# hellojialee/OffsetGuided

Measured on AMD Instinct MI355X. Metric: images/sec end-to-end (backbone+decode) @640x640 bs8; decoder-only ms/img, higher is better.
Workload: dtype f16

## Files before the change

### offsetguided_amd/csrc/conv3x3.hip

```cpp
#include <stdio.h>
#include <stdlib.h>

#include <type_traits>

#include "lp_dtype.h"
#include "og_common.h"

namespace {

typedef lp8 bf16x8;
typedef float f32x4 __attribute__((ext_vector_type(4)));
typedef unsigned short u16x4 __attribute__((ext_vector_type(4)));
typedef unsigned short u16x8 __attribute__((ext_vector_type(8)));

constexpr int kZeroPageBytes = 256;

struct ConvArgs {
    const unsigned short *x;
    const unsigned short *w;
    const float *bias;
    const unsigned short *skip;
    unsigned short *out;
    unsigned short *up;
    float *partial;
    int *counters;
    const unsigned short *zero;
    int N, H, W, Cin, Cout, M;
    int Hin, Win, stride, taps;
    int n_tiles, steps_per_split, ksplit, relu;
    const unsigned short *x2;
    int Cin2, H2, W2, stride2, steps_main, steps_total, w_row;
    uint32_t magic_w, magic_h, magic_chunks;
    int x_bytes, w_bytes;
    unsigned long long *stamps;
    OgWarm warm;
};

#if defined(OG_TILED_STAMPS) || defined(OG_PW_STAMPS)
#ifndef OG_DEBUG_STAMPS
#define OG_DEBUG_STAMPS 1
#endif
#endif
#ifdef OG_DEBUG_STAMPS
#define CONV_STAMP(i)                                                                                         \
    do {                                                                                                      \
        if (a.stamps && tid == 0)                                                                             \
            a.stamps[((size_t)blockIdx.y * gridDim.x + blockIdx.x) * 8 + (i)] = __builtin_amdgcn_s_memrealtime(); \
    } while (0)
#else
#define CONV_STAMP(i) do { } while (0)
#endif

__device__ __forceinline__ unsigned short f2bf(float f) { return f2lp(f); }
__device__ __forceinline__ float bf2f(unsigned short u) { return lp2f(u); }

__device__ __forceinline__ void glds16(const void *g, unsigned char *l)
{
    __builtin_amdgcn_global_load_lds((const __attribute__((address_space(1))) void *)g,
                                     (__attribute__((address_space(3))) void *)l, 16, 0, 0);
}

__device__ __forceinline__ void blds16(__amdgpu_buffer_rsrc_t r, uint32_t voff, uint32_t soff, unsigned char *l)
{
    __builtin_amdgcn_raw_ptr_buffer_load_lds(r, (__attribute__((address_space(3))) void *)l, 16, voff, soff, 0, 0);
}
constexpr uint32_t kOobOffset = 0x80000000u;

__device__ __forceinline__ void store_b128_sc1(__amdgpu_buffer_rsrc_t r, uint32_t voff, uint32_t soff, f32x4 v)
{
    asm volatile("buffer_store_dwordx4 %0, %1, %2, %3 offen sc1\n\ts_nop 1" ::"v"(v), "v"(voff), "s"(r), "s"(soff) : "memory");
}

template <int N>
__device__ __forceinline__ void wait_vm_lgkm0()
{
    __builtin_amdgcn_s_waitcnt((N & 15) | (7 << 4) | (0 << 8) | ((N >> 4) << 14));
    asm volatile("" ::: "memory");
}

__device__ __forceinline__ uint32_t div_magic(uint32_t n, uint32_t magic) { return magic ? __umulhi(n, magic) : n; }

template <int BM, int BN>
struct EpiloguePre {
    f32x4 bias[BN / 32];
    u16x4 skip[BM / 32][BN / 32];
};

template <int BM, int BN>
__device__ __forceinline__ void epilogue_load(EpiloguePre<BM, BN> &pre, const ConvArgs &a, int m0, int n0, int wave, int lane)
{
    constexpr int MT = BM / 32, NT = BN / 32;
    const int wm = wave >> 1, wn = wave & 1;
#pragma unroll
    for (int n = 0; n < NT; ++n)
        pre.bias[n] = *reinterpret_cast<const f32x4 *>(a.bias + n0 + wn * (BN / 2) + n * 16 + (lane >> 4) * 4);
#pragma unroll
    for (int m = 0; m < MT; ++m) {
        const int pm = m0 + wm * (BM / 2) + m * 16 + (lane & 15);
#pragma unroll
        for (int n = 0; n < NT; ++n) {
            const int co = n0 + wn * (BN / 2) + n * 16 + (lane >> 4) * 4;
            pre.skip[m][n] = (u16x4){0, 0, 0, 0};
            if (a.skip && pm < a.M) pre.skip[m][n] = *reinterpret_cast<const u16x4 *>(a.skip + (size_t)pm * a.Cout + co);
        }
    }
}

template <int BM, int BN>
__device__ __forceinline__ void epilogue_finish(const f32x4 (&acc)[BN / 32][BM / 32], const EpiloguePre<BM, BN> &pre,
                                                const ConvArgs &a, int m0, int n0, int wave, int lane)
{
    constexpr int MT = BM / 32, NT = BN / 32;
    const int wm = wave >> 1, wn = wave & 1;
#pragma unroll
    for (int m = 0; m < MT; ++m) {
        const int pm = m0 + wm * (BM / 2) + m * 16 + (lane & 15);
        if (pm >= a.M) continue;
#pragma unroll
// ... 446 lines not shown
    OG_REQUIRE(x2, OG_EINVAL, "og_conv2d_proj: null pointer");
    Proj pj;
    pj.x2 = x2; pj.H2 = H2; pj.W2 = W2; pj.Cin2 = Cin2; pj.stride2 = stride2;
    return conv_run(OG_LP_STR("og_conv2d_proj"), x, w_cat, bias, nullptr, out, N, Hin, Win, Cin, Cout, ksize, stride, relu, workspace,
                    workspace_bytes, stream, pj);
}

#ifndef OG_DT_F16
OG_API int og_conv3x3s2_tiled_supported(int N, int H, int W, int Cin, int Cout)
{
    if (N <= 0 || H <= 0 || W <= 0 || Cin <= 0 || Cout <= 0 || (H & 1) || (W & 1)) return 0;
    if ((long)N * H * W * Cin >= (1l << 30) || (long)N * H * W * Cout >= (1l << 32)) return 0;
    if (Cout % 128 || Cin % 64) return 0;
    return ((H / 2) % 8 == 0 && (W / 2) % 16 == 0) ? 1 : ((W / 2) == 40 && (H / 2) % 2 == 0) ? 2 : 0;
}

OG_API int og_conv3x3_tiled_supported(int N, int H, int W, int Cin, int Cout)
{
    if (N <= 0 || H <= 0 || W <= 0 || Cin <= 0 || Cout <= 0) return 0;
    if ((long)N * H * W * Cin >= (1l << 30) || (long)N * H * W * Cout >= (1l << 30)) return 0;
    return tiled_kind(H, W, Cin, Cout);
}

OG_API size_t og_conv3x3_tiled_workspace_bytes(int N, int H, int W, int Cin, int Cout)
{
    const int kind = og_conv3x3_tiled_supported(N, H, W, Cin, Cout);
    if (!kind) return 0;
    const long items = tiled_items(kind, N, H, W, Cout);
    const int ks = tiled_ksplit(kind, items, Cin);
    if (ks <= 1 || items > (long)kMaxTiles) return 0;
    return kZeroPageBytes + kMaxTiles * sizeof(int) + (size_t)items * ks * tiled_slab_bytes(kind);
}

OG_API int og_conv3x3_pack_w16(const void *w, int Cin, int Cout, int order, void *packed, void *stream)
{
    OG_REQUIRE(order >= 0 && order <= 3, OG_EINVAL,
               "og_conv3x3_pack_w16: order is 0 / 1 (3x3, stride 1 / 2) or 2 / 3 (1x1, cout tiles of 128 / 64)");
    OG_REQUIRE(w && packed, OG_EINVAL, "og_conv3x3_pack_w16: null pointer");
    OG_REQUIRE(Cin > 0 && Cout > 0 && Cin % 64 == 0 && Cout % (order == 3 ? 64 : 128) == 0, OG_EUNSUPPORTED,
               "og_conv3x3_pack_w16: Cin must be a multiple of 64 and Cout of %d (got %d -> %d)", order == 3 ? 64 : 128, Cin, Cout);
    const long slots = (long)Cout * (order >= 2 ? 1 : 9) * Cin / 8;
    hipLaunchKernelGGL(conv3x3_pack_kernel, dim3((unsigned)((slots + 255) / 256)), dim3(256), 0, (hipStream_t)stream,
                       (const unsigned short *)w, (unsigned short *)packed, Cin, Cout, order);
    OG_LAUNCH_CHECK("og_conv3x3_pack_w16");
    return OG_OK;
}
#endif

namespace {
int conv3x3_tiled_impl(const char *name, const void *x, const void *w_packed, const float *bias, const void *skip, void *out, void *up,
                       int N, int H, int W, int Cin, int Cout, int relu, void *workspace, size_t workspace_bytes, void *stream)
{
    const OgWarm warm = og_take_warm_hint();
    OG_REQUIRE(x && w_packed && bias && (out || up), OG_EINVAL, "%s: null pointer", name);
    OG_REQUIRE(!up || (uintptr_t)up % 16 == 0, OG_EINVAL, "%s: `up` must be 16-byte aligned", name);
    OG_REQUIRE(N > 0 && H > 0 && W > 0, OG_EINVAL, "%s: bad shape", name);
    const long M = (long)N * H * W;
    OG_REQUIRE(M * (long)Cin < (1l << 30) && M * (long)Cout < (1l << 30), OG_EUNSUPPORTED, "%s: tensor too large (>= 2 GiB)", name);
    const int kind = tiled_kind(H, W, Cin, Cout);
    OG_REQUIRE(kind != 0, OG_EUNSUPPORTED, "%s: needs Cout %% 128 == 0, Cin %% 64 == 0 and H, W multiples of 16 or W == 40 with H %% 4 == 0 "
               "(got %dx%d, %d -> %d)", name, H, W, Cin, Cout);
    ConvArgs h = {};
    h.x = (const unsigned short *)x; h.w = (const unsigned short *)w_packed; h.bias = bias;
    h.skip = (const unsigned short *)skip; h.out = (unsigned short *)out; h.up = (unsigned short *)up;
    h.N = N; h.H = H; h.W = W; h.Cin = Cin; h.Cout = Cout; h.M = (int)M; h.n_tiles = Cout / 128; h.relu = relu;
    h.Hin = H; h.Win = W; h.stride = 1; h.taps = 9;
    h.x_bytes = (int)(M * Cin * 2);
    h.w_bytes = Cout * 9 * Cin * 2;
#ifdef OG_TILED_STAMPS
    h.stamps = g_stamps;
#endif
    hipStream_t st = (hipStream_t)stream;
    h.warm = warm;
    const long items = tiled_items(kind, N, H, W, Cout);
    h.ksplit = (items <= (long)kMaxTiles) ? tiled_ksplit(kind, items, Cin) : 1;
    if (h.ksplit > 1) {
        const size_t need = kZeroPageBytes + kMaxTiles * sizeof(int) + (size_t)items * h.ksplit * tiled_slab_bytes(kind);
        OG_REQUIRE(workspace && workspace_bytes >= need, OG_ENOSPC, "%s: workspace %zu < %zu bytes (og_conv3x3_tiled_workspace_bytes)", name,
                   workspace ? workspace_bytes : (size_t)0, need);
        OG_REQUIRE((uintptr_t)workspace % 256 == 0, OG_EINVAL, "%s: workspace must be 256-byte aligned", name);
        h.counters = (int *)((char *)workspace + kZeroPageBytes);
        h.partial = (float *)((char *)workspace + kZeroPageBytes + kMaxTiles * sizeof(int));
    }
#define TILED_LAUNCH(TW_, TH_, WM_, VAR_)                                                                             \
    do {                                                                                                              \
        constexpr int halo_ = ((TW_ + 2) * (TH_ + 2) * 5 * 16 + 1023) / 1024 * 1024;                                  \
        const int lds_ = 2 * halo_ + (TW_ == 20 ? OG_TILED_RING20 : TW_ == 40 ? OG_TILED_RING40 : 3) * 128 * 64 + 1024; \
        static OgAttrOnce attr_;                                                                                      \
        if (attr_.need())                                                                                             \
            (void)hipFuncSetAttribute((const void *)conv3x3_tiled_kernel<TW_, TH_, WM_, VAR_, 4>,                     \
                                      hipFuncAttributeMaxDynamicSharedMemorySize, 160 * 1024);                        \
        const long blocks_ = (long)N * (H / TH_) * (W / TW_) * h.n_tiles * h.ksplit;                                  \
        hipLaunchKernelGGL((conv3x3_tiled_kernel<TW_, TH_, WM_, VAR_, 4>), dim3((unsigned)blocks_), dim3(256), lds_, st, h); \
    } while (0)
#ifndef OG_TILED_VAR16
#define OG_TILED_VAR16 26
#endif
    if (kind == 1) TILED_LAUNCH(16, 16, 4, OG_TILED_VAR16);
    else if (kind == 3) TILED_LAUNCH(20, 4, 1, 2);
    else TILED_LAUNCH(40, 4, 2, 2);
#undef TILED_LAUNCH
    OG_LAUNCH_CHECK(name);
    return OG_OK;
}
}

OG_API int OG_LP_NAME(og_conv3x3_tiled)(const void *x, const void *w_packed, const float *bias, const void *skip, void *out, int N,
                                        int H, int W, int Cin, int Cout, int relu, void *workspace, size_t workspace_bytes,
                                        void *stream)
{
    return conv3x3_tiled_impl(OG_LP_STR("og_conv3x3_tiled"), x, w_packed, bias, skip, out, nullptr, N, H, W, Cin, Cout, relu, workspace,
                              workspace_bytes, stream);
}

OG_API int OG_LP_NAME(og_conv3x3_tiled_up2)(const void *x, const void *w_packed, const float *bias, const void *skip, void *up, int N,
                                            int H, int W, int Cin, int Cout, int relu, void *workspace, size_t workspace_bytes,
                                            void *stream)
{
    const char *name = OG_LP_STR("og_conv3x3_tiled_up2");
    OG_REQUIRE(up, OG_EINVAL, "%s: null pointer", name);
    OG_REQUIRE((long)N * H * W * 4 * Cout < (1l << 30), OG_EUNSUPPORTED, "%s: tensor too large (>= 2 GiB)", name);
    return conv3x3_tiled_impl(name, x, w_packed, bias, skip, nullptr, up, N, H, W, Cin, Cout, relu, workspace, workspace_bytes, stream);
}

OG_API int OG_LP_NAME(og_conv3x3s2_tiled)(const void *x, const void *w_packed, const float *bias, const void *skip, void *out,
                                          int N, int Hin, int Win, int Cin, int Cout, int relu, void *stream)
{
    const char *name = OG_LP_STR("og_conv3x3s2_tiled");
    OG_REQUIRE(x && w_packed && bias && out, OG_EINVAL, "%s: null pointer", name);
    OG_REQUIRE(N > 0 && Hin > 0 && Win > 0 && !(Hin & 1) && !(Win & 1), OG_EINVAL, "%s: bad shape", name);
    const int H = Hin / 2, W = Win / 2;
    const long M = (long)N * H * W, Min = (long)N * Hin * Win;
    OG_REQUIRE(Min * (long)Cin < (1l << 30) && M * (long)Cout < (1l << 30), OG_EUNSUPPORTED, "%s: tensor too large (>= 2 GiB)", name);
    const int kind = og_conv3x3s2_tiled_supported(N, Hin, Win, Cin, Cout);
    OG_REQUIRE(kind != 0, OG_EUNSUPPORTED,
               "%s: needs Cout %% 128 == 0, Cin %% 64 == 0 and an output of 8k x 16k pixels or 2k x 40 (got %dx%d -> %dx%d, %d -> %d)", name,
               Hin, Win, H, W, Cin, Cout);
    ConvArgs h = {};
    h.warm = og_take_warm_hint();
    h.x = (const unsigned short *)x; h.w = (const unsigned short *)w_packed; h.bias = bias;
    h.skip = (const unsigned short *)skip; h.out = (unsigned short *)out;
    h.N = N; h.H = H; h.W = W; h.Cin = Cin; h.Cout = Cout; h.M = (int)M; h.n_tiles = Cout / 128; h.relu = relu;
    h.Hin = Hin; h.Win = Win; h.stride = 2; h.taps = 9;
    h.x_bytes = (int)(Min * Cin * 2);
    h.w_bytes = Cout * 9 * Cin * 2;
    constexpr int lds_ = 3 * 128 * 64 + 3 * 3 * 4096;
#define S2_LAUNCH(TW_, TH_, WM_, VAR_)                                                                                \
    do {                                                                                                              \
        static OgAttrOnce attr_;                                                                                      \
        if (attr_.need())                                                                                             \
            (void)hipFuncSetAttribute((const void *)conv3x3s2_tiled_kernel<TW_, TH_, WM_, VAR_>,                      \
                                      hipFuncAttributeMaxDynamicSharedMemorySize, lds_);                              \
        const long blocks_ = (long)N * (H / TH_) * (W / TW_) * h.n_tiles;                                             \
        hipLaunchKernelGGL((conv3x3s2_tiled_kernel<TW_, TH_, WM_, VAR_>), dim3((unsigned)blocks_), dim3(256), lds_,   \
                           (hipStream_t)stream, h);                                                                   \
    } while (0)
    if (kind == 2) S2_LAUNCH(40, 2, 1, 2);
    else S2_LAUNCH(16, 8, 2, 2);
#undef S2_LAUNCH
    OG_LAUNCH_CHECK(name);
    return OG_OK;
}

static int pw_fill(const char *name, PwArgs &a, const void *x1, int C1, int H1, int W1, int s1, const void *x2, int C2, int H2, int W2,
                   int s2, const void *w_packed, const float *bias, int N, int H, int W, int Cout, int bn)
{
    OG_REQUIRE(x1 && w_packed, OG_EINVAL, "%s: null pointer", name);
    OG_REQUIRE(N > 0 && H > 0 && W > 0 && (s1 == 1 || s1 == 2) && (!x2 || s2 == 1 || s2 == 2), OG_EINVAL, "%s: bad shape", name);
    OG_REQUIRE(C1 > 0 && C1 % 64 == 0 && (!x2 || (C2 > 0 && C2 % 64 == 0)) && Cout % bn == 0, OG_EUNSUPPORTED,
               "%s: input channels must be multiples of 64 and Cout of %d (got %d + %d -> %d)", name, bn, C1, x2 ? C2 : 0, Cout);
    OG_REQUIRE((H - 1) * s1 < H1 && (W - 1) * s1 < W1, OG_EINVAL, "%s: the strided output reaches outside the input", name);
    OG_REQUIRE(!x2 || (C2 == C1 && H2 == H1 && W2 == W1 && s2 == s1), OG_EUNSUPPORTED,
               "%s: a second input must have the shape and stride of the first", name);
    const long M = (long)N * H * W;
    OG_REQUIRE((long)N * H1 * W1 * C1 < (1l << 30) && (!x2 || (long)N * H2 * W2 * C2 < (1l << 30)) && M * Cout < (1l << 30), OG_EUNSUPPORTED,
// ... 82 lines not shown
```

### offsetguided_amd/csrc/conv3x3_tiled.inc

```

template <int N, int I = 0, class F>
__device__ __forceinline__ void og_static_for(F &&f)
{
    if constexpr (I < N) {
        f(std::integral_constant<int, I>());
        og_static_for<N, I + 1>(f);
    }
}

__host__ __device__ __forceinline__ constexpr int tiled_swz(int row) { return (4 - ((row >> 2) & 3)) & 3; }

__global__ void __launch_bounds__(256)
conv3x3_pack_kernel(const unsigned short *w, unsigned short *packed, int Cin, int Cout, int order)
{
    const long slot = (long)blockIdx.x * 256 + threadIdx.x;
    const int taps = order >= 2 ? 1 : 9, rows = order == 3 ? 64 : 128;
    const long total = (long)Cout * taps * Cin / 8;
    if (slot >= total) return;
    const int chunks = Cin >> 5;
    const int in_stage = (int)(slot % (rows * 4));
    long stage = slot / (rows * 4);
    const int kS2[9] = {0, 2, 6, 8, 3, 5, 1, 7, 4};
    const int tslot = (int)(stage % taps), tap = order == 1 ? kS2[tslot] : tslot;
    stage /= taps;
    const int q = (int)(stage % chunks), nt = (int)(stage / chunks);
    const int r = in_stage >> 2, jp = in_stage & 3, j = jp ^ tiled_swz(r);
    const unsigned short *src = w + ((size_t)(nt * rows + r) * taps + tap) * Cin + q * 32;
    u16x8 v;
#pragma unroll
    for (int e = 0; e < 8; ++e) v[e] = src[order >= 2 ? 8 * j + e : (e < 4 ? 4 * j + e : 16 + 4 * j + (e - 4))];
    *reinterpret_cast<u16x8 *>(packed + slot * 8) = v;
}

template <int TW, int TH, int WM, int VAR, int NW>
__device__ __forceinline__ void conv3x3_tiled_body(const ConvArgs &a, const int bid, const int nblk)
{
    constexpr int BN = 128, WN = NW / WM, kThr = 64 * NW, kPieceB = kThr * 16;
    constexpr int kHaloW = TW + 2, kHaloPx = (TW + 2) * (TH + 2), kPitch = 80;
    constexpr int NPA = (kHaloPx * 5 + kThr - 1) / kThr;
    constexpr int kABytes = (kHaloPx * 5 * 16 + 1023) / 1024 * 1024, kBBytes = BN * 64;
#ifndef OG_TILED_RING20
#define OG_TILED_RING20 6
#endif
#ifndef OG_TILED_RING40
#define OG_TILED_RING40 4
#endif
    constexpr int kRing = TW == 20 ? OG_TILED_RING20 : TW == 40 ? OG_TILED_RING40 : 3;
    constexpr bool kWfRot = TW == 16 && (VAR & 16) != 0;
    constexpr bool kWfAhead = kRing > 3 || kWfRot;
    constexpr int kAhead = kWfAhead ? kRing : kRing - 1;
    constexpr int kWin = kWfAhead ? kAhead - 2 : kAhead - 1;
    static_assert(kRing == 3 || kRing == 4 || kRing == 6 || kRing == 9, "ring sizes the slot arithmetic serves");
    constexpr int kDump = kRing * kBBytes + 2 * kABytes;
    constexpr int PW = kBBytes / kPieceB;
    constexpr int MT = TW * TH / 16 / WM, NT = 8 / WN;
    static_assert(TW * TH % (16 * WM) == 0 && NW % WM == 0 && 8 % WN == 0 && PW >= 1, "unsupported tile");
    static_assert(NPA <= 8 - kWin, "the last halo piece must be older than everything tap 8's wait leaves in flight (the steps 8 - kWin .. 7)");
    static_assert(kDump + 1024 <= 80 * 1024, "two workgroups per CU");
    extern __shared__ __attribute__((aligned(1024))) unsigned char lds[];
    unsigned char *const bufB = lds, *const bufA = lds + kRing * kBBytes;

    const int tid = threadIdx.x, wave = tid >> 6, lane = tid & 63;
    const unsigned warm_v = og_warm_touch(a.warm, (unsigned)bid * kThr + (unsigned)tid);
#ifdef OG_TILED_STAMPS
    {
        unsigned long long rt_entry;
        asm volatile("s_memrealtime %0\n\ts_waitcnt lgkmcnt(0)" : "=s"(rt_entry));
        if (a.stamps) a.stamps[((size_t)blockIdx.x * 4 + wave) * 16 + 7] = rt_entry;
    }
#endif
    const int wid = ((nblk & 7) == 0 && !(VAR & 4)) ? og_xcd_remap(bid, nblk) : bid;
    const int ksplit = a.ksplit, item = wid / ksplit, split = wid - item * ksplit;
    const int tiles_x = a.W / TW, tiles_y = a.H / TH, chunks = a.Cin >> 5;
    const int q0 = split * (chunks / ksplit), q_end = q0 + chunks / ksplit;
    const int nt_i = item % a.n_tiles;
    int t = item / a.n_tiles;
    const int tx = t % tiles_x;
    t /= tiles_x;
    const int ty = t % tiles_y, img = t / tiles_y;
    const int n0 = nt_i * BN;

    const __amdgpu_buffer_rsrc_t xr = __builtin_amdgcn_make_buffer_rsrc(const_cast<unsigned short *>(a.x), 0, a.x_bytes, 0x00020000);
    const __amdgpu_buffer_rsrc_t wr = __builtin_amdgcn_make_buffer_rsrc(const_cast<unsigned short *>(a.w), 0, a.w_bytes, 0x00020000);
    uint32_t a_off[NPA];
#pragma unroll
    for (int i = 0; i < NPA; ++i) {
        const int p = tid + kThr * i, hp = p / 5, c = p - hp * 5;
        const int hy = hp / kHaloW, hx = hp - hy * kHaloW;
        const int gy = ty * TH - 1 + hy, gx = tx * TW - 1 + hx;
        const bool ok = c < 4 && hp < kHaloPx && gy >= 0 && gy < a.H && gx >= 0 && gx < a.W;
        a_off[i] = ok ? (uint32_t)((((img * a.H + gy) * a.W + gx) * a.Cin + c * 8) * 2) : kOobOffset;
    }
    const int piece = wave * 64 * 16;
    const uint32_t w_voff = (uint32_t)tid * 16;
    const uint32_t w_tile = (uint32_t)nt_i * (uint32_t)(chunks * 9 * kBBytes);
    auto issue_a = [&](int i, int q, int buf) {
        const int blk = i * kPieceB + piece;
        blds16(xr, a_off[i], q * 64, blk < kABytes ? bufA + buf * kABytes + blk : lds + kDump);
    };
    int ring_lo = 0, ring_hi = 2 * kBBytes;
    auto ring_off = [&](int slot) { return kRing == 4 ? (slot < 2 ? ring_lo : ring_hi) + (slot & 1) * kBBytes : slot * kBBytes; };
    auto issue_b = [&](int step, int ring_bytes) {
#pragma unroll
        for (int i = 0; i < PW; ++i)
            blds16(wr, w_voff, w_tile + step * kBBytes + i * kPieceB, bufB + ring_bytes + piece + i * kPieceB);
    };

    const int wm = wave / WN, wn = wave % WN;
    const int fcol = lane & 15, fk = lane >> 4;
    const int w_rd = ((wn * NT) * 16 + fcol) * 64 + ((fk ^ tiled_swz(fcol)) << 4);
    int px_off[MT];
#pragma unroll
    for (int m = 0; m < MT; ++m) {
        const int lp = (wm * MT + m) * 16 + fcol;
        px_off[m] = ((lp / TW) * kHaloW + lp % TW) * kPitch + fk * 8;
    }

    typedef unsigned long long u64;
    typedef u64 u64x2 __attribute__((ext_vector_type(2)));
    const uint32_t lds_a = (uint32_t)(uintptr_t)(__attribute__((address_space(3))) unsigned char *)bufA;
    uint32_t px_addr[TW == 16 ? 1 : MT];
#pragma unroll
    for (int m = 0; m < (TW == 16 ? 1 : MT); ++m) px_addr[m] = lds_a + px_off[m];
    auto read_px1 = [&](auto m_tag, auto off_tag, uint32_t buf_off, bf16x8 (&pf)[MT]) {
        constexpr int OFF = decltype(off_tag)::value, m = decltype(m_tag)::value;
        constexpr int imm = OFF + (TW == 16 ? m * kHaloW * kPitch : 0);
        const uint32_t addr = px_addr[TW == 16 ? 0 : m] + buf_off;
        u64 lo, hi;
        asm volatile("ds_read_b64 %0, %1 offset:%2" : "=v"(lo) : "v"(addr), "i"(imm));
        asm volatile("ds_read_b64 %0, %1 offset:%2" : "=v"(hi) : "v"(addr), "i"(imm + 32));
        u64x2 v;
        v[0] = lo;
        v[1] = hi;
        pf[m] = __builtin_bit_cast(bf16x8, v);
    };
    auto read_px = [&](auto off_tag, uint32_t buf_off, bf16x8 (&pf)[MT]) {
        og_static_for<MT>([&](auto m_tag) { read_px1(m_tag, off_tag, buf_off, pf); });
    };

    f32x4 acc[NT][MT];
    if (a.skip && split == 0) {
        static_assert(NT % 2 == 0, "cout blocks in pairs");
        u16x8 sk2[NT / 2][MT];
#pragma unroll
        for (int m = 0; m < MT; ++m) {
            const int lp = (wm * MT + m) * 16 + fcol;
            const size_t opx = (size_t)(img * a.H + ty * TH + lp / TW) * a.W + tx * TW + lp % TW;
#pragma unroll
            for (int np = 0; np < NT / 2; ++np)
                sk2[np][m] = __builtin_nontemporal_load(reinterpret_cast<const u16x8 *>(a.skip + opx * a.Cout + n0 + (wn * NT + 2 * np + (fk & 1)) * 16 + (fk >> 1) * 8));
        }
#pragma unroll
        for (int i = 0; i < NPA; ++i) issue_a(i, q0, 0);
#pragma unroll
        for (int i = 0; i < kAhead; ++i) issue_b(9 * q0 + i, (i % kRing) * kBBytes);
#pragma unroll
        for (int np = 0; np < NT / 2; ++np)
#pragma unroll
            for (int m = 0; m < MT; ++m) {
                typedef uint32_t u32x4s __attribute__((ext_vector_type(4)));
                typedef uint32_t u32x2s __attribute__((ext_vector_type(2)));
                const u32x4s v = __builtin_bit_cast(u32x4s, sk2[np][m]);
                const auto r0 = __builtin_amdgcn_permlane16_swap(v[0], v[2], false, false);
                const auto r1 = __builtin_amdgcn_permlane16_swap(v[1], v[3], false, false);
                const u16x4 lo = __builtin_bit_cast(u16x4, (u32x2s){r0[0], r1[0]}), hi = __builtin_bit_cast(u16x4, (u32x2s){r0[1], r1[1]});
                acc[2 * np][m] = (f32x4){bf2f(lo[0]), bf2f(lo[1]), bf2f(lo[2]), bf2f(lo[3])};
                acc[2 * np + 1][m] = (f32x4){bf2f(hi[0]), bf2f(hi[1]), bf2f(hi[2]), bf2f(hi[3])};
            }
    } else {
#pragma unroll
        for (int i = 0; i < NPA; ++i) issue_a(i, q0, 0);
#pragma unroll
        for (int i = 0; i < kAhead; ++i) issue_b(9 * q0 + i, (i % kRing) * kBBytes);
#pragma unroll
        for (int n = 0; n < NT; ++n)
#pragma unroll
            for (int m = 0; m < MT; ++m) acc[n][m] = (f32x4){0.f, 0.f, 0.f, 0.f};
    }

    constexpr int kSets = NT == 8 ? 9 : NT == 4 ? 6 : 3, kFree = kSets - NT;
    static_assert(!kWfRot || ((18 * NT) % kSets == 0 && kFree >= 1 && NT * (MT - 1) >= kFree + 1 + MT), "rotating fragment sets");
    bf16x8 pf[2][MT], wf[kWfAhead && !kWfRot ? 2 : 1][kWfRot ? kSets : NT];
#ifdef OG_TILED_STAMPS
    unsigned long long st_end, st_w, st_b, st_prev;
    uint32_t sum_wait = 0, sum_bar = 0, sum_body = 0, n_st = 0;
    {
        unsigned long long mt0, rt0;
        asm volatile("s_memtime %0\n\ts_memrealtime %1\n\ts_waitcnt lgkmcnt(0)" : "=s"(mt0), "=s"(rt0));
        st_end = st_w = st_b = st_prev = mt0;
        if (a.stamps) {
            a.stamps[((size_t)blockIdx.x * 4 + wave) * 16 + 4] = mt0;
            a.stamps[((size_t)blockIdx.x * 4 + wave) * 16 + 5] = rt0;
        }
    }
#endif
    wait_vm_lgkm0<(kAhead - 1) * PW>();
    __builtin_amdgcn_s_barrier();
    asm volatile("" ::: "memory");
#ifdef OG_TILED_STAMPS
    {
        unsigned long long rt_first;
        asm volatile("s_memrealtime %0\n\ts_waitcnt lgkmcnt(0)" : "=s"(rt_first));
        if (a.stamps) a.stamps[((size_t)blockIdx.x * 4 + wave) * 16 + 9] = rt_first;
    }
#endif
    read_px(std::integral_constant<int, 0>(), 0u, pf[0]);
    if constexpr (kWfAhead) {
#pragma unroll
        for (int n = 0; n < NT; ++n) wf[0][n] = *reinterpret_cast<const bf16x8 *>(bufB + w_rd + n * 1024);
    }

    auto chunk_body = [&](auto more_tag, auto par_tag, int q) {
        constexpr bool MORE = decltype(more_tag)::value;
        constexpr int PAR = decltype(par_tag)::value;
        const uint32_t cur_off = (uint32_t)((q & 1) * kABytes), nxt_off = (uint32_t)(((q + 1) & 1) * kABytes);
        og_static_for<9>([&](auto tap_tag) {
            constexpr int tap = decltype(tap_tag)::value;
            constexpr int kSlot0 = kRing == 6 ? 3 * PAR : kRing == 4 ? PAR : 0;
            const int s = q * 9 + tap;
            {
                constexpr int kYounger = [] {
                    int n = 0;
                    for (int j = 1; j <= kWin; ++j) {
                        const int t = tap - j;
                        if (t < 0) n += PW;
                        else n += ((MORE && t < NPA) ? 1 : 0) + ((MORE || t + kAhead < 9) ? PW : 0);
                    }
                    return n;
                }();
                wait_vm_lgkm0<kYounger>();
            }
#ifdef OG_TILED_STAMPS
            asm volatile("" : "+s"(st_end), "+s"(st_w), "+s"(st_b));
            sum_wait += (uint32_t)st_w - (uint32_t)st_prev;
            sum_bar += (uint32_t)st_b - (uint32_t)st_w;
            sum_body += (uint32_t)st_end - (uint32_t)st_b;
            st_prev = st_end;
            ++n_st;
            asm volatile("s_memtime %0" : "=s"(st_w));
#endif
            __builtin_amdgcn_s_barrier();
#ifdef OG_TILED_STAMPS
            asm volatile("s_memtime %0" : "=s"(st_b));
#endif
            __builtin_amdgcn_sched_barrier(0);
            auto issue_dma = [&]() {
                if (MORE && tap < NPA) issue_a(tap, q + 1, (q + 1) & 1);
                if (MORE || tap + kAhead < 9) issue_b(s + kAhead, ring_off((kSlot0 + tap + kAhead) % kRing));
            };
            const unsigned char *wB = bufB + ring_off((kSlot0 + tap + (kWfAhead ? 1 : 0)) % kRing);
            constexpr int wcur = kWfAhead ? (PAR + tap) & 1 : 0, wnxt = kWfAhead ? (PAR + tap + 1) & 1 : 0;
            if constexpr (kWfRot) {
                constexpr bool kNext = MORE || tap < 8;
                constexpr int t18 = PAR * 9 + tap, cur = (PAR + tap) & 1, nxt = cur ^ 1;
                if (!(VAR & 1)) __builtin_amdgcn_s_setprio(1);
                og_static_for<NT * MT>([&](auto i_tag) {
                    constexpr int i = decltype(i_tag)::value, n = i / MT, m = i % MT;
                    acc[n][m] = OG_LP_MFMA(wf[0][(t18 * NT + n) % kSets], pf[cur][m], acc[n][m]);
                    if constexpr (m == MT - 1) {
                        constexpr int j = n + kFree;
                        if constexpr (j < NT && kNext)
                            wf[0][((t18 + 1) * NT + j) % kSets] = *reinterpret_cast<const bf16x8 *>(wB + w_rd + j * 1024);
                    } else {
                        constexpr int k = n * (MT - 1) + m;
                        if constexpr (k < kFree) {
                            if constexpr (kNext) wf[0][((t18 + 1) * NT + k) % kSets] = *reinterpret_cast<const bf16x8 *>(wB + w_rd + k * 1024);
                        } else if constexpr (k == kFree) {
                            issue_dma();
                        } else if constexpr (k - kFree - 1 < MT) {
                            constexpr int pm = k - kFree - 1;
                            if constexpr (tap < 8)
                                read_px1(std::integral_constant<int, pm>(), std::integral_constant<int, (((tap + 1) / 3) * kHaloW + (tap + 1) % 3) * kPitch>(),
                                         cur_off, pf[nxt]);
                            else if constexpr (MORE)
                                read_px1(std::integral_constant<int, pm>(), std::integral_constant<int, 0>(), nxt_off, pf[nxt]);
                        }
                    }
                    __builtin_amdgcn_sched_barrier(0);
                });
                if (!(VAR & 1)) __builtin_amdgcn_s_setprio(0);
            } else if constexpr (kWfAhead) {
                static_assert(NT * MT >= 1 + MT + NT, "an MFMA gap per issue item");
                constexpr bool kNext = MORE || tap < 8;
                constexpr int cur = (PAR + tap) & 1, nxt = cur ^ 1;
                if (!(VAR & 1)) __builtin_amdgcn_s_setprio(1);
                og_static_for<NT * MT>([&](auto i_tag) {
                    constexpr int i = decltype(i_tag)::value, n = i / MT, m = i % MT;
                    acc[n][m] = OG_LP_MFMA(wf[wcur][n], pf[cur][m], acc[n][m]);
                    if constexpr (i == 0) {
                        issue_dma();
                    } else if constexpr (i - 1 < MT) {
                        if constexpr (tap < 8)
                            read_px1(std::integral_constant<int, i - 1>(), std::integral_constant<int, (((tap + 1) / 3) * kHaloW + (tap + 1) % 3) * kPitch>(),
                                     cur_off, pf[nxt]);
                        else if constexpr (MORE)
                            read_px1(std::integral_constant<int, i - 1>(), std::integral_constant<int, 0>(), nxt_off, pf[nxt]);
                    } else if constexpr (i - 1 - MT < NT) {
                        if constexpr (kNext) wf[wnxt][i - 1 - MT] = *reinterpret_cast<const bf16x8 *>(wB + w_rd + (i - 1 - MT) * 1024);
                    }
                    __builtin_amdgcn_sched_barrier(0);
                });
                if (!(VAR & 1)) __builtin_amdgcn_s_setprio(0);
            } else {
            if (!(VAR & 2)) issue_dma();
            if constexpr (tap < 8)
                read_px(std::integral_constant<int, (((tap + 1) / 3) * kHaloW + (tap + 1) % 3) * kPitch>(), cur_off, pf[(PAR + tap + 1) & 1]);
            else if constexpr (MORE)
                read_px(std::integral_constant<int, 0>(), nxt_off, pf[(PAR + tap + 1) & 1]);
#pragma unroll
            for (int n = 0; n < NT; ++n) wf[0][n] = *reinterpret_cast<const bf16x8 *>(wB + w_rd + n * 1024);
            if (VAR & 2) issue_dma();
            if (!(VAR & 1)) __builtin_amdgcn_s_setprio(1);
#pragma unroll
            for (int n = 0; n < NT; ++n)
#pragma unroll
                for (int m = 0; m < MT; ++m) acc[n][m] = OG_LP_MFMA(wf[wcur][n], pf[(PAR + tap) & 1][m], acc[n][m]);
            if (!(VAR & 1)) __builtin_amdgcn_s_setprio(0);
            }
#ifdef OG_TILED_STAMPS
            asm volatile("s_memtime %0" : "=s"(st_end));
#endif
        });
    };
    const std::true_type yes;
    const std::false_type no;
    const std::integral_constant<int, 0> even;
    const std::integral_constant<int, 1> odd;
    int q = q0;
#pragma unroll 1
    for (; q + 2 < q_end; q += 2) {
        chunk_body(yes, even, q);
        chunk_body(yes, odd, q + 1);
        if constexpr (kRing == 4) {
            const int t = ring_lo;
            ring_lo = ring_hi;
            ring_hi = t;
        }
    }
    chunk_body(yes, even, q);
    chunk_body(no, odd, q + 1);

#ifdef OG_TILED_STAMPS
    {
        unsigned long long mt1, rt1;
        asm volatile("s_waitcnt lgkmcnt(0)\n\ts_memtime %0\n\ts_memrealtime %1\n\ts_waitcnt lgkmcnt(0)" : "=s"(mt1), "=s"(rt1));
        asm volatile("" : "+s"(st_end), "+s"(st_w), "+s"(st_b));
        sum_wait += (uint32_t)st_w - (uint32_t)st_prev;
        sum_bar += (uint32_t)st_b - (uint32_t)st_w;
        sum_body += (uint32_t)st_end - (uint32_t)st_b;
        if (a.stamps && lane == 0) {
            unsigned long long *o = a.stamps + ((size_t)blockIdx.x * 4 + wave) * 16;
            o[0] = sum_wait; o[1] = sum_bar; o[2] = sum_body; o[3] = n_st; o[12] = mt1; o[6] = rt1;
            o[10] = __builtin_amdgcn_s_getreg((4) | (0 << 6) | (31 << 11));
            o[11] = __builtin_amdgcn_s_getreg((20) | (0 << 6) | (31 << 11));
        }
    }
#endif
    if (ksplit > 1) {
        typedef uint32_t u32x4 __attribute__((ext_vector_type(4)));
        constexpr int F = NT * MT;
        constexpr uint32_t kSlabBytes = F * kThr * 16;
        uint64_t slab_base = reinterpret_cast<uint64_t>(a.partial) + (uint64_t)item * ksplit * kSlabBytes;
        slab_base = ((uint64_t)(uint32_t)__builtin_amdgcn_readfirstlane((int)(slab_base >> 32)) << 32) |
                    (uint64_t)(uint32_t)__builtin_amdgcn_readfirstlane((int)(uint32_t)slab_base);
        const __amdgpu_buffer_rsrc_t slabs = __builtin_amdgcn_make_buffer_rsrc(
            reinterpret_cast<char *>(slab_base), 0, __builtin_amdgcn_readfirstlane((int)(ksplit * kSlabBytes)), 0x00020000);
        const uint32_t own_off = __builtin_amdgcn_readfirstlane(split * kSlabBytes);
#pragma unroll
        for (int n = 0; n < NT; ++n)
#pragma unroll
            for (int m = 0; m < MT; ++m)
                store_b128_sc1(slabs, (n * MT + m) * kThr * 16 + tid * 16, own_off, acc[n][m]);
        asm volatile("s_waitcnt vmcnt(0)" ::: "memory");
        __syncthreads();
        int *flag = reinterpret_cast<int *>(lds);
        if (tid == 0) {
            const int old = __hip_atomic_fetch_add(a.counters + item, 1, __ATOMIC_RELAXED, __HIP_MEMORY_SCOPE_AGENT);
            const int last = old == ksplit - 1;
            if (last) __hip_atomic_store(a.counters + item, 0, __ATOMIC_RELAXED, __HIP_MEMORY_SCOPE_AGENT);
            *flag = last;
        }
        __syncthreads();
        if (!*flag) return;
#pragma unroll
        for (int n = 0; n < NT; ++n)
#pragma unroll
            for (int m = 0; m < MT; ++m) acc[n][m] = (f32x4){0.f, 0.f, 0.f, 0.f};
        for (int sp = 0; sp < ksplit; ++sp) {
            const uint32_t soff = __builtin_amdgcn_readfirstlane(sp * kSlabBytes);
            f32x4 part[F];
#pragma unroll
            for (int i = 0; i < F; ++i)
                part[i] = __builtin_bit_cast(f32x4, __builtin_amdgcn_raw_buffer_load_b128(slabs, i * kThr * 16 + tid * 16, soff, 16));
#pragma unroll
            for (int n = 0; n < NT; ++n)
#pragma unroll
                for (int m = 0; m < MT; ++m) acc[n][m] += part[n * MT + m];
        }
    }

    constexpr int kOPitch = BN * 2 + 16, kTilePx = TW * TH, kPerPx = BN / 8;
    static_assert(kTilePx * kOPitch <= kDump + 1024, "output staging must fit the LDS of the main loop");
    f32x4 bias_r[NT];
#pragma unroll
    for (int n = 0; n < NT; ++n) bias_r[n] = *reinterpret_cast<const f32x4 *>(a.bias + n0 + (wn * NT + n) * 16 + fk * 4);
    __syncthreads();
#pragma unroll
    for (int m = 0; m < MT; ++m) {
        const int px = (wm * MT + m) * 16 + fcol;
#pragma unroll
        for (int n = 0; n < NT; ++n) {
            const int cl = (wn * NT + n) * 16 + fk * 4;
            const f32x4 v = acc[n][m] + bias_r[n];
            u16x4 o;
#pragma unroll
            for (int jj = 0; jj < 4; ++jj) o[jj] = f2bf(a.relu ? fmaxf(v[jj], 0.f) : v[jj]);
            *reinterpret_cast<u16x4 *>(lds + px * kOPitch + cl * 2) = o;
        }
    }
    __syncthreads();
    if (a.up) {
        const int W2 = 2 * a.W;
        const size_t up_tile = ((size_t)img * 2 * a.H + 2 * ty * TH) * W2 + 2 * tx * TW;
        constexpr int kPieces = kTilePx * kPerPx;
        static_assert(kPieces % kThr == 0, "whole rounds");
        for (int g0 = tid; g0 < kPieces; g0 += 2 * kThr) {
            u16x8 lo[2], hi[2][4];
            size_t off[2];
#pragma unroll
            for (int u = 0; u < 2; ++u) {
                const int g = min(g0 + u * kThr, kPieces - kThr + tid), px = g / kPerPx, cg = g % kPerPx;
                off[u] = (up_tile + (size_t)(2 * (px / TW)) * W2 + 2 * (px % TW)) * a.Cout + n0 + cg * 8;
#pragma unroll
                for (int q = 0; q < 4; ++q)
                    hi[u][q] = *reinterpret_cast<const u16x8 *>(a.up + off[u] + ((size_t)(q >> 1) * W2 + (q & 1)) * a.Cout);
                lo[u] = *reinterpret_cast<const u16x8 *>(lds + px * kOPitch + cg * 16);
            }
#pragma unroll
            for (int u = 0; u < 2; ++u)
#pragma unroll
                for (int q = 0; q < 4; ++q) {
                    if (u == 1 && g0 + kThr >= kPieces) continue;
                    u16x8 o;
#pragma unroll
                    for (int j = 0; j < 8; ++j) o[j] = f2bf(bf2f(hi[u][q][j]) + bf2f(lo[u][j]));
                    *reinterpret_cast<u16x8 *>(a.up + off[u] + ((size_t)(q >> 1) * W2 + (q & 1)) * a.Cout) = o;
                }
        }
    } else {
        const size_t tile_px = (size_t)(img * a.H + ty * TH) * a.W + tx * TW;
        for (int g = tid; g < kTilePx * kPerPx; g += kThr) {
            const int px = g / kPerPx, cg = g % kPerPx;
            const size_t off = (tile_px + (size_t)(px / TW) * a.W + (px % TW)) * a.Cout + n0 + cg * 8;
            *reinterpret_cast<u16x8 *>(a.out + off) = *reinterpret_cast<const u16x8 *>(lds + px * kOPitch + cg * 16);
        }
    }
#ifdef OG_TILED_STAMPS
    if (a.stamps && lane == 0) {
        unsigned long long rt_end;
        asm volatile("s_memrealtime %0\n\ts_waitcnt lgkmcnt(0)" : "=s"(rt_end));
        a.stamps[((size_t)blockIdx.x * 4 + wave) * 16 + 8] = rt_end;
    }
#endif
    og_warm_sink(warm_v);
}

template <int TW, int TH, int WM, int VAR = 0, int NW = 4>
__global__ void __launch_bounds__(64 * NW, NW / 2)
conv3x3_tiled_kernel(ConvArgs a)
{
    conv3x3_tiled_body<TW, TH, WM, VAR, NW>(a, blockIdx.x, gridDim.x);
}

template <int TW, int TH, int WM, int VAR = 0>
__global__ void __launch_bounds__(256, 2)
conv3x3s2_tiled_kernel(ConvArgs a)
{
    constexpr int BN = 128, WN = 4 / WM;
    constexpr bool kRowFrag = TW == 16;
    constexpr int kPitch = 80, kImgPx = (TW + 1) * (TH + 1);
    constexpr int NPA = (kImgPx * 5 + 255) / 256;
    constexpr int kABytes = NPA * 256 * 16, kBBytes = BN * 64, kRing = 3;
    constexpr int PW = kBBytes / (256 * 16);
    constexpr int MT = TW * TH / 16 / WM, NT = 8 / WN;
    static_assert(TW * TH % (16 * WM) == 0 && 4 % WM == 0, "unsupported tile");
    static_assert(NPA == 3, "the static halo schedule below issues three pieces per phase image");
    static_assert(kRing * kBBytes + 3 * kABytes <= 80 * 1024, "two workgroups per CU");
    extern __shared__ __attribute__((aligned(1024))) unsigned char lds[];
    unsigned char *const bufB = lds, *const bufA = lds + kRing * kBBytes;

    const int tid = threadIdx.x, wave = tid >> 6, lane = tid & 63;
    const unsigned warm_v = og_warm_touch(a.warm, blockIdx.x * 256u + (unsigned)tid);
    const int nblk = gridDim.x;
    const int item = (nblk & 7) == 0 ? og_xcd_remap(blockIdx.x, nblk) : blockIdx.x;
    const int tiles_x = a.W / TW, tiles_y = a.H / TH, chunks = a.Cin >> 5;
    const int nt_i = item % a.n_tiles;
    int t_ = item / a.n_tiles;
    const int tx = t_ % tiles_x;
    t_ /= tiles_x;
    const int ty = t_ % tiles_y, img = t_ / tiles_y;
    const int n0 = nt_i * BN, y0 = ty * TH, x0 = tx * TW;

    const __amdgpu_buffer_rsrc_t xr = __builtin_amdgcn_make_buffer_rsrc(const_cast<unsigned short *>(a.x), 0, a.x_bytes, 0x00020000);
    const __amdgpu_buffer_rsrc_t wr = __builtin_amdgcn_make_buffer_rsrc(const_cast<unsigned short *>(a.w), 0, a.w_bytes, 0x00020000);
    uint32_t a_off[4][NPA];
#pragma unroll
    for (int p = 0; p < 4; ++p) {
        const int odd_r = (p == 0 || p == 2), odd_c = (p == 0 || p == 1);
        const int pw = TW + odd_c, phh = TH + odd_r;
#pragma unroll
        for (int i = 0; i < NPA; ++i) {
            const int sl = tid + 256 * i, hp = sl / 5, c = sl - hp * 5;
            const int ri = hp / pw, ci = hp - ri * pw;
            const int iy = 2 * (y0 + ri) - odd_r, ix = 2 * (x0 + ci) - odd_c;
            const bool ok = c < 4 && ri < phh && iy >= 0 && iy < a.Hin && ix >= 0 && ix < a.Win;
            a_off[p][i] = ok ? (uint32_t)((((img * a.Hin + iy) * a.Win + ix) * a.Cin + c * 8) * 2) : kOobOffset;
        }
    }
    const int piece = wave * 64 * 16;
    const uint32_t w_voff = (uint32_t)tid * 16;
    const uint32_t w_tile = (uint32_t)nt_i * (uint32_t)(chunks * 9 * kBBytes);
    auto issue_h = [&](int p, int i, int q, uint32_t buf_off) { blds16(xr, a_off[p][i], q * 64, bufA + buf_off + piece + i * 4096); };
    auto issue_b = [&](int step, int ring) {
#pragma unroll
        for (int i = 0; i < PW; ++i)
            blds16(wr, w_voff, w_tile + step * kBBytes + i * 4096, bufB + ring * kBBytes + piece + i * 4096);
    };

    const int wm = wave / WN, wn = wave % WN;
    const int fcol = lane & 15, fk = lane >> 4;
    const int w_rd = ((wn * NT) * 16 + fcol) * 64 + ((fk ^ tiled_swz(fcol)) << 4);
    typedef unsigned long long u64;
    typedef u64 u64x2 __attribute__((ext_vector_type(2)));
    const uint32_t lds_a = (uint32_t)(uintptr_t)(__attribute__((address_space(3))) unsigned char *)bufA;
    uint32_t pxE[kRowFrag ? 1 : MT], pxO[kRowFrag ? 1 : MT];
#pragma unroll
    for (int m = 0; m < (kRowFrag ? 1 : MT); ++m) {
        const int tp = (wm * MT + m) * 16 + fcol, r = tp / TW, c = tp - r * TW;
        pxE[m] = lds_a + (uint32_t)((r * TW + c) * kPitch + fk * 8);
        pxO[m] = lds_a + (uint32_t)((r * (TW + 1) + c) * kPitch + fk * 8);
    }
    auto read_px1 = [&](auto m_tag, auto pw_tag, auto off_tag, uint32_t buf_off, bf16x8 (&pf)[MT]) {
        constexpr int PWID = decltype(pw_tag)::value, OFF = decltype(off_tag)::value, m = decltype(m_tag)::value;
        constexpr int imm = OFF + (kRowFrag ? m * PWID * kPitch : 0);
        const uint32_t addr = (PWID == TW ? pxE[kRowFrag ? 0 : m] : pxO[kRowFrag ? 0 : m]) + buf_off;
        u64 lo, hi;
        asm volatile("ds_read_b64 %0, %1 offset:%2" : "=v"(lo) : "v"(addr), "i"(imm));
// ... 390 lines not shown
```

Before: 1521.

## Issue weight prefetch before tile index math and precompute magic divisors

Moves the first weight-ring loads ahead of the tile coordinate decode so global loads start earlier, and replaces runtime integer divisions for ksplit/n_tiles/tiles_x/tiles_y with host-precomputed magic-number multiplies. Skip-tensor loads and halo loads are hoisted and interleaved with offset computation, and the prologue wait now drains all loads. Epilogue thread-index values are recomputed behind an asm barrier to shorten register live ranges. The full drain before the first barrier may lose some overlap that the partial wait previously allowed.

```diff
diff --git a/offsetguided_amd/csrc/conv3x3.hip b/offsetguided_amd/csrc/conv3x3.hip
--- a/offsetguided_amd/csrc/conv3x3.hip
+++ b/offsetguided_amd/csrc/conv3x3.hip
@@ -34,6 +34,9 @@
     int x_bytes, w_bytes;
     unsigned long long *stamps;
     OgWarm warm;
+    int tiles_x, tiles_y, chunks_split;
+    uint32_t magic_ksplit, magic_ntiles, magic_tx, magic_ty;
+    uint32_t w_tile_bytes;
 };
 
 #if defined(OG_TILED_STAMPS) || defined(OG_PW_STAMPS)
@@ -646,6 +649,10 @@
         h.counters = (int *)((char *)workspace + kZeroPageBytes);
         h.partial = (float *)((char *)workspace + kZeroPageBytes + kMaxTiles * sizeof(int));
     }
+    auto magic = [](uint32_t d) { return d <= 1 ? 0u : (uint32_t)(((1ull << 32) + d - 1) / d); };
+    h.chunks_split = (Cin >> 5) / h.ksplit;
+    h.magic_ksplit = magic((uint32_t)h.ksplit); h.magic_ntiles = magic((uint32_t)h.n_tiles);
+    h.w_tile_bytes = (uint32_t)(Cin >> 5) * 9u * (128u * 64u);
 #define TILED_LAUNCH(TW_, TH_, WM_, VAR_)                                                                             \
     do {                                                                                                              \
         constexpr int halo_ = ((TW_ + 2) * (TH_ + 2) * 5 * 16 + 1023) / 1024 * 1024;                                  \
@@ -655,6 +662,8 @@
             (void)hipFuncSetAttribute((const void *)conv3x3_tiled_kernel<TW_, TH_, WM_, VAR_, 4>,                     \
                                       hipFuncAttributeMaxDynamicSharedMemorySize, 160 * 1024);                        \
         const long blocks_ = (long)N * (H / TH_) * (W / TW_) * h.n_tiles * h.ksplit;                                  \
+        h.tiles_x = W / TW_; h.tiles_y = H / TH_;                                                                     \
+        h.magic_tx = magic((uint32_t)h.tiles_x); h.magic_ty = magic((uint32_t)h.tiles_y);                             \
         hipLaunchKernelGGL((conv3x3_tiled_kernel<TW_, TH_, WM_, VAR_, 4>), dim3((unsigned)blocks_), dim3(256), lds_, st, h); \
     } while (0)
 #ifndef OG_TILED_VAR16
diff --git a/offsetguided_amd/csrc/conv3x3_tiled.inc b/offsetguided_amd/csrc/conv3x3_tiled.inc
--- a/offsetguided_amd/csrc/conv3x3_tiled.inc
+++ b/offsetguided_amd/csrc/conv3x3_tiled.inc
@@ -70,44 +70,81 @@
     }
 #endif
     const int wid = ((nblk & 7) == 0 && !(VAR & 4)) ? og_xcd_remap(bid, nblk) : bid;
-    const int ksplit = a.ksplit, item = wid / ksplit, split = wid - item * ksplit;
-    const int tiles_x = a.W / TW, tiles_y = a.H / TH, chunks = a.Cin >> 5;
-    const int q0 = split * (chunks / ksplit), q_end = q0 + chunks / ksplit;
-    const int nt_i = item % a.n_tiles;
-    int t = item / a.n_tiles;
-    const int tx = t % tiles_x;
-    t /= tiles_x;
-    const int ty = t % tiles_y, img = t / tiles_y;
-    const int n0 = nt_i * BN;
-
-    const __amdgpu_buffer_rsrc_t xr = __builtin_amdgcn_make_buffer_rsrc(const_cast<unsigned short *>(a.x), 0, a.x_bytes, 0x00020000);
+    const int ksplit = a.ksplit, item = (int)div_magic((uint32_t)wid, a.magic_ksplit), split = wid - item * ksplit;
+    const int q0 = split * a.chunks_split, q_end = q0 + a.chunks_split;
+    int t = (int)div_magic((uint32_t)item, a.magic_ntiles);
+    const int nt_i = item - t * a.n_tiles, n0 = nt_i * BN;
+
     const __amdgpu_buffer_rsrc_t wr = __builtin_amdgcn_make_buffer_rsrc(const_cast<unsigned short *>(a.w), 0, a.w_bytes, 0x00020000);
-    uint32_t a_off[NPA];
-#pragma unroll
-    for (int i = 0; i < NPA; ++i) {
-        const int p = tid + kThr * i, hp = p / 5, c = p - hp * 5;
-        const int hy = hp / kHaloW, hx = hp - hy * kHaloW;
-        const int gy = ty * TH - 1 + hy, gx = tx * TW - 1 + hx;
-        const bool ok = c < 4 && hp < kHaloPx && gy >= 0 && gy < a.H && gx >= 0 && gx < a.W;
-        a_off[i] = ok ? (uint32_t)((((img * a.H + gy) * a.W + gx) * a.Cin + c * 8) * 2) : kOobOffset;
-    }
     const int piece = wave * 64 * 16;
     const uint32_t w_voff = (uint32_t)tid * 16;
-    const uint32_t w_tile = (uint32_t)nt_i * (uint32_t)(chunks * 9 * kBBytes);
+    const uint32_t w_tile = (uint32_t)nt_i * a.w_tile_bytes;
+    int ring_lo = 0, ring_hi = 2 * kBBytes;
+    auto ring_off = [&](int slot) { return kRing == 4 ? (slot < 2 ? ring_lo : ring_hi) + (slot & 1) * kBBytes : slot * kBBytes; };
+    auto issue_b = [&](int step, int ring_bytes) {
+#pragma unroll
+        for (int i = 0; i < PW; ++i)
+            blds16(wr, w_voff, w_tile + step * kBBytes + i * kPieceB, bufB + ring_bytes + piece + i * kPieceB);
+    };
+#ifdef OG_TILED_STAMPS
+    {
+        unsigned long long rt_req0;
+        __builtin_amdgcn_sched_barrier(0);
+        asm volatile("s_memrealtime %0\n\ts_waitcnt lgkmcnt(0)" : "=s"(rt_req0));
+        if (a.stamps) a.stamps[((size_t)blockIdx.x * 4 + wave) * 16 + 13] = rt_req0;
+        __builtin_amdgcn_sched_barrier(0);
+    }
+#endif
+#pragma unroll
+    for (int i = 0; i < kAhead; ++i) issue_b(9 * q0 + i, (i % kRing) * kBBytes);
+
+    const int t_img = (int)div_magic((uint32_t)t, a.magic_tx), tx = t - t_img * a.tiles_x;
+    const int img = (int)div_magic((uint32_t)t_img, a.magic_ty), ty = t_img - img * a.tiles_y;
+    const int wm = wave / WN, wn = wave % WN;
+    const int fcol = lane & 15, fk = lane >> 4;
+
+    static_assert(NT % 2 == 0, "cout blocks in pairs");
+    const bool has_skip = a.skip && split == 0;
+    u16x8 sk2[NT / 2][MT];
+    if (has_skip) {
+#pragma unroll
+        for (int m = 0; m < MT; ++m) {
+            const int lp = (wm * MT + m) * 16 + fcol;
+            const size_t opx = (size_t)(img * a.H + ty * TH + lp / TW) * a.W + tx * TW + lp % TW;
+#pragma unroll
+            for (int np = 0; np < NT / 2; ++np)
+                sk2[np][m] = __builtin_nontemporal_load(reinterpret_cast<const u16x8 *>(a.skip + opx * a.Cout + n0 + (wn * NT + 2 * np + (fk & 1)) * 16 + (fk >> 1) * 8));
+        }
+    }
+
+    const __amdgpu_buffer_rsrc_t xr = __builtin_amdgcn_make_buffer_rsrc(const_cast<unsigned short *>(a.x), 0, a.x_bytes, 0x00020000);
+    uint32_t a_off[NPA];
     auto issue_a = [&](int i, int q, int buf) {
         const int blk = i * kPieceB + piece;
         blds16(xr, a_off[i], q * 64, blk < kABytes ? bufA + buf * kABytes + blk : lds + kDump);
     };
-    int ring_lo = 0, ring_hi = 2 * kBBytes;
-    auto ring_off = [&](int slot) { return kRing == 4 ? (slot < 2 ? ring_lo : ring_hi) + (slot & 1) * kBBytes : slot * kBBytes; };
-    auto issue_b = [&](int step, int ring_bytes) {
-#pragma unroll
-        for (int i = 0; i < PW; ++i)
-            blds16(wr, w_voff, w_tile + step * kBBytes + i * kPieceB, bufB + ring_bytes + piece + i * kPieceB);
-    };
-
-    const int wm = wave / WN, wn = wave % WN;
-    const int fcol = lane & 15, fk = lane >> 4;
+    {
+        const int gy0 = ty * TH - 1, gx0 = tx * TW - 1, row0 = img * a.H;
+#pragma unroll
+        for (int i = 0; i < NPA; ++i) {
+            const int p = tid + kThr * i, hp = p / 5, c = p - hp * 5;
+            const int hy = hp / kHaloW, hx = hp - hy * kHaloW;
+            const int gy = gy0 + hy, gx = gx0 + hx;
+            const bool ok = c < 4 && hp < kHaloPx && gy >= 0 && gy < a.H && gx >= 0 && gx < a.W;
+            a_off[i] = ok ? (uint32_t)((((row0 + gy) * a.W + gx) * a.Cin + c * 8) * 2) : kOobOffset;
+            issue_a(i, q0, 0);
+        }
+    }
+    __builtin_amdgcn_sched_barrier(0);
+#ifdef OG_TILED_STAMPS
+    {
+        unsigned long long rt_req1;
+        asm volatile("s_memrealtime %0\n\ts_waitcnt lgkmcnt(0)" : "=s"(rt_req1));
+        if (a.stamps) a.stamps[((size_t)blockIdx.x * 4 + wave) * 16 + 14] = rt_req1;
+        __builtin_amdgcn_sched_barrier(0);
+    }
+#endif
+
     const int w_rd = ((wn * NT) * 16 + fcol) * 64 + ((fk ^ tiled_swz(fcol)) << 4);
     int px_off[MT];
 #pragma unroll
@@ -139,21 +176,7 @@
     };
 
     f32x4 acc[NT][MT];
-    if (a.skip && split == 0) {
-        static_assert(NT % 2 == 0, "cout blocks in pairs");
-        u16x8 sk2[NT / 2][MT];
-#pragma unroll
-        for (int m = 0; m < MT; ++m) {
-            const int lp = (wm * MT + m) * 16 + fcol;
-            const size_t opx = (size_t)(img * a.H + ty * TH + lp / TW) * a.W + tx * TW + lp % TW;
-#pragma unroll
-            for (int np = 0; np < NT / 2; ++np)
-                sk2[np][m] = __builtin_nontemporal_load(reinterpret_cast<const u16x8 *>(a.skip + opx * a.Cout + n0 + (wn * NT + 2 * np + (fk & 1)) * 16 + (fk >> 1) * 8));
-        }
-#pragma unroll
-        for (int i = 0; i < NPA; ++i) issue_a(i, q0, 0);
-#pragma unroll
-        for (int i = 0; i < kAhead; ++i) issue_b(9 * q0 + i, (i % kRing) * kBBytes);
+    if (has_skip) {
 #pragma unroll
         for (int np = 0; np < NT / 2; ++np)
 #pragma unroll
@@ -168,10 +191,6 @@
                 acc[2 * np + 1][m] = (f32x4){bf2f(hi[0]), bf2f(hi[1]), bf2f(hi[2]), bf2f(hi[3])};
             }
     } else {
-#pragma unroll
-        for (int i = 0; i < NPA; ++i) issue_a(i, q0, 0);
-#pragma unroll
-        for (int i = 0; i < kAhead; ++i) issue_b(9 * q0 + i, (i % kRing) * kBBytes);
 #pragma unroll
         for (int n = 0; n < NT; ++n)
 #pragma unroll
@@ -194,7 +213,8 @@
         }
     }
 #endif
-    wait_vm_lgkm0<(kAhead - 1) * PW>();
+    wait_vm_lgkm0<0>();
+    og_warm_sink(warm_v);
     __builtin_amdgcn_s_barrier();
     asm volatile("" ::: "memory");
 #ifdef OG_TILED_STAMPS
@@ -356,6 +376,10 @@
         }
     }
 #endif
+    int tid_e = tid;
+    asm volatile("" : "+v"(tid_e));
+    const int wave_e = tid_e >> 6, lane_e = tid_e & 63, wm_e = wave_e / WN, wn_e = wave_e % WN, fcol_e = lane_e & 15, fk_e = lane_e >> 4;
+    (void)lane_e;
     if (ksplit > 1) {
         typedef uint32_t u32x4 __attribute__((ext_vector_type(4)));
         constexpr int F = NT * MT;
@@ -370,11 +394,11 @@
         for (int n = 0; n < NT; ++n)
 #pragma unroll
             for (int m = 0; m < MT; ++m)
-                store_b128_sc1(slabs, (n * MT + m) * kThr * 16 + tid * 16, own_off, acc[n][m]);
+                store_b128_sc1(slabs, (n * MT + m) * kThr * 16 + tid_e * 16, own_off, acc[n][m]);
         asm volatile("s_waitcnt vmcnt(0)" ::: "memory");
         __syncthreads();
         int *flag = reinterpret_cast<int *>(lds);
-        if (tid == 0) {
+        if (tid_e == 0) {
             const int old = __hip_atomic_fetch_add(a.counters + item, 1, __ATOMIC_RELAXED, __HIP_MEMORY_SCOPE_AGENT);
             const int last = old == ksplit - 1;
             if (last) __hip_atomic_store(a.counters + item, 0, __ATOMIC_RELAXED, __HIP_MEMORY_SCOPE_AGENT);
@@ -391,7 +415,7 @@
             f32x4 part[F];
 #pragma unroll
             for (int i = 0; i < F; ++i)
-                part[i] = __builtin_bit_cast(f32x4, __builtin_amdgcn_raw_buffer_load_b128(slabs, i * kThr * 16 + tid * 16, soff, 16));
+                part[i] = __builtin_bit_cast(f32x4, __builtin_amdgcn_raw_buffer_load_b128(slabs, i * kThr * 16 + tid_e * 16, soff, 16));
 #pragma unroll
             for (int n = 0; n < NT; ++n)
 #pragma unroll
@@ -403,14 +427,14 @@
     static_assert(kTilePx * kOPitch <= kDump + 1024, "output staging must fit the LDS of the main loop");
     f32x4 bias_r[NT];
 #pragma unroll
-    for (int n = 0; n < NT; ++n) bias_r[n] = *reinterpret_cast<const f32x4 *>(a.bias + n0 + (wn * NT + n) * 16 + fk * 4);
+    for (int n = 0; n < NT; ++n) bias_r[n] = *reinterpret_cast<const f32x4 *>(a.bias + n0 + (wn_e * NT + n) * 16 + fk_e * 4);
     __syncthreads();
 #pragma unroll
     for (int m = 0; m < MT; ++m) {
-        const int px = (wm * MT + m) * 16 + fcol;
+        const int px = (wm_e * MT + m) * 16 + fcol_e;
 #pragma unroll
         for (int n = 0; n < NT; ++n) {
-            const int cl = (wn * NT + n) * 16 + fk * 4;
+            const int cl = (wn_e * NT + n) * 16 + fk_e * 4;
             const f32x4 v = acc[n][m] + bias_r[n];
             u16x4 o;
 #pragma unroll
@@ -424,12 +448,12 @@
         const size_t up_tile = ((size_t)img * 2 * a.H + 2 * ty * TH) * W2 + 2 * tx * TW;
         constexpr int kPieces = kTilePx * kPerPx;
         static_assert(kPieces % kThr == 0, "whole rounds");
-        for (int g0 = tid; g0 < kPieces; g0 += 2 * kThr) {
+        for (int g0 = tid_e; g0 < kPieces; g0 += 2 * kThr) {
             u16x8 lo[2], hi[2][4];
             size_t off[2];
 #pragma unroll
             for (int u = 0; u < 2; ++u) {
-                const int g = min(g0 + u * kThr, kPieces - kThr + tid), px = g / kPerPx, cg = g % kPerPx;
+                const int g = min(g0 + u * kThr, kPieces - kThr + tid_e), px = g / kPerPx, cg = g % kPerPx;
                 off[u] = (up_tile + (size_t)(2 * (px / TW)) * W2 + 2 * (px % TW)) * a.Cout + n0 + cg * 8;
 #pragma unroll
                 for (int q = 0; q < 4; ++q)
@@ -449,20 +473,19 @@
         }
     } else {
         const size_t tile_px = (size_t)(img * a.H + ty * TH) * a.W + tx * TW;
-        for (int g = tid; g < kTilePx * kPerPx; g += kThr) {
+        for (int g = tid_e; g < kTilePx * kPerPx; g += kThr) {
             const int px = g / kPerPx, cg = g % kPerPx;
             const size_t off = (tile_px + (size_t)(px / TW) * a.W + (px % TW)) * a.Cout + n0 + cg * 8;
             *reinterpret_cast<u16x8 *>(a.out + off) = *reinterpret_cast<const u16x8 *>(lds + px * kOPitch + cg * 16);
         }
     }
 #ifdef OG_TILED_STAMPS
-    if (a.stamps && lane == 0) {
+    if (a.stamps && lane_e == 0) {
         unsigned long long rt_end;
         asm volatile("s_memrealtime %0\n\ts_waitcnt lgkmcnt(0)" : "=s"(rt_end));
-        a.stamps[((size_t)blockIdx.x * 4 + wave) * 16 + 8] = rt_end;
-    }
-#endif
-    og_warm_sink(warm_v);
+        a.stamps[((size_t)blockIdx.x * 4 + wave_e) * 16 + 8] = rt_end;
+    }
+#endif
 }
 
 template <int TW, int TH, int WM, int VAR = 0, int NW = 4>
```

Result: slower. 1467 (-3.6%).
